# suilin0432/SoS-WSOD

Measured on AMD Instinct MI355X. Metric: images/s (1/2/4/8 MI355X) VGG16+OICR 2000-prop; conv5_3 MFMA-util %, higher is better.
Workload: dtype bf16; 1 GPU; OICR+ training iteration: 4 views/step/GPU (1 image(s) x 2 scales x h-flip, every view 512x512), R=2000 proposals/view, K=20, VGG16 dilated-C5 + ROIPool 7x7 + fc6/fc7 4096 + WSDDN + 4 OICR heads, fwd+bwd+SGD(momentum, wd); image=one view, parallelism=dp1

## Files before the change

### include/soswsod_hip.h

```cpp
#ifndef SOSWSOD_HIP_H
#define SOSWSOD_HIP_H

#include <stdint.h>

#ifdef __cplusplus
extern "C" {
#endif

#ifndef SW_F32
#define SW_F32 0
#define SW_BF16 1
#endif

typedef struct ihipStream_t* sw_stream_t;

typedef struct sw_epilogue {
  const float* bias;
  int relu;
  const uint8_t* drop_mask;
  long ld_drop;
  float drop_scale;
  const void* relu_ref;
  long ld_ref;
  float ref_scale;
  int ref_dtype;
  int out_dtype;
  int accumulate_atomic;
  float* absmax_out;
  uint64_t drop_seed, drop_offset;
  float drop_hash_p;
  const uint64_t* drop_offset_dev;
  float* splitk_workspace;
  const void* residual;
  long ld_res;
  int res_dtype;
  const float* fold_row_scale;
  const struct sw_sgd_tensor_s* sgd_fused;
  float sgd_momentum, sgd_grad_scale;
} sw_epilogue;

int sw_gemm(int dtype, int a_kstrided, int b_kstrided, int M, int N, int K, const void* A, long lda, const void* B,
            long ldb, void* C, long ldc, const sw_epilogue* ep, int splitk, sw_stream_t stream);
long sw_gemm_splitk_workspace_floats(int M, int N, int K, int splitk);

int sw_conv3x3_igemm(int dtype, int nimg, int H, int W, int Cin, int Cout, int dilation, const void* in,
                     const void* wk, void* out, const sw_epilogue* ep, sw_stream_t stream);
int sw_conv3x3_relu_pool2(int dtype, int nimg, int H, int W, int Cin, int Cout, const void* in, const void* wk, const float* bias,
                          void* out_pooled, sw_stream_t stream);
typedef struct sw_conv_problem {
  int32_t nimg, H, W, Cin, Cout;
  const void* in; const void* wk; void* out;
  const sw_epilogue* ep;
} sw_conv_problem;
int sw_conv3x3_multi(int dtype, int n, const sw_conv_problem* probs, sw_stream_t stream);
long sw_conv3x3_wgrad_workspace_floats(int dtype, int nimg, int H, int W, int Cin, int Cout, int splitk);
int sw_conv3x3_wgrad(int dtype, int nimg, int H, int W, int Cin, int Cout, int dilation, const void* x,
                     const void* dy, float* dw_oihw, float* workspace, int splitk, sw_stream_t stream);
int sw_conv3x3_wgrad_scaled(int dtype, int nimg, int H, int W, int Cin, int Cout, int dilation, const void* x, const void* dy,
                            float* dw_oihw, float* workspace, int splitk, const float* cout_scale, sw_stream_t stream);
int sw_conv3x3_wgrad_acc(int dtype, int nimg, int H, int W, int Cin, int Cout, int dilation, const void* x, const void* dy,
                         float* dw_oihw, float* workspace, int splitk, const float* cout_scale, int accumulate, sw_stream_t stream);
int sw_conv3x3_wgrad_small(int dtype, int nimg, int H, int W, int Cin, int Cout, const void* x, const void* dy,
                           const float* cout_scale, float* dw_oihw, sw_stream_t stream);
int sw_conv3x3_wgrad_small_acc(int dtype, int nimg, int H, int W, int Cin, int Cout, const void* x, const void* dy,
                               const float* cout_scale, float* dw_oihw, int accumulate, sw_stream_t stream);
int sw_conv3x3_wgrad_slabs(int dtype, int nimg, int H, int W, int Cin, int Cout, int dilation, const void* x,
                           const void* dy, float* workspace, int splitk, sw_stream_t stream);
int sw_conv3x3_wgrad_fold(int Cin, int Cout, int nslab, const float* workspace, float* dw_oihw, sw_stream_t stream);
int sw_conv3x3_wgrad_fold_acc(int Cin, int Cout, int nslab, const float* workspace, float* dw_oihw, const float* cout_scale,
                              int accumulate, sw_stream_t stream);
typedef struct {
  int nimg, H, W, Cin, Cout, dilation, nsplit;
  const void* x;
  const void* dy;
  float* slabs;
} sw_wgrad_problem;
int sw_conv3x3_wgrad_grouped(int dtype, int n_problems, const sw_wgrad_problem* problems, sw_stream_t stream);
typedef struct sw_gemm_kk_problem {
  const void* A; const void* B; float* slabs;
  int32_t M, N, K, nsplit;
  long lda, ldb;
} sw_gemm_kk_problem;
int sw_gemm_kk_grouped(int dtype, int n_problems, const sw_gemm_kk_problem* problems, sw_stream_t stream);
long sw_gemm_kk_grouped_slabs(int dtype, int K, int nsplit);
typedef struct sw_splitk_fold { int32_t M, N, nslab, accumulate; const float* workspace; float* C; long ldc; const float* row_scale; } sw_splitk_fold;
int sw_splitk_fold_multi(int n, const sw_splitk_fold* folds, sw_stream_t stream);
typedef struct { int Cin, Cout, nslab; const float* workspace; float* dw_oihw; } sw_wgrad_fold;
int sw_conv3x3_wgrad_fold_multi(int n, const sw_wgrad_fold* folds, sw_stream_t stream);
int sw_conv_weight_prep(int dtype, int mode, int Cout, int Cin, int cin_pad, const float* w_oihw, void* wk,
                        sw_stream_t stream);

int sw_maxpool2x2_fwd(int dtype, int nimg, int H, int W, int C, int stride, const void* in, void* out,
                      sw_stream_t stream);
int sw_maxpool2x2_bwd(int dtype, int nimg, int H, int W, int C, int stride, const void* in, const void* dout,
                      void* din, int relu_mask, sw_stream_t stream);
// ... 260 lines not shown
```

### sos-wsod_amd/_lib.py

```python
import ctypes
import os

import torch

_HERE = os.path.dirname(os.path.abspath(__file__))
LIB_PATH = os.environ.get("SW_LIB_PATH") or os.path.join(_HERE, "libsoswsod_hip.so")

SW_F32, SW_BF16 = 0, 1

c_int, c_long, c_float, c_void_p, c_u64 = ctypes.c_int, ctypes.c_long, ctypes.c_float, ctypes.c_void_p, ctypes.c_uint64


class Epilogue(ctypes.Structure):
    _fields_ = [
        ("bias", c_void_p), ("relu", c_int), ("drop_mask", c_void_p), ("ld_drop", c_long), ("drop_scale", c_float),
        ("relu_ref", c_void_p), ("ld_ref", c_long), ("ref_scale", c_float), ("ref_dtype", c_int),
        ("out_dtype", c_int), ("accumulate_atomic", c_int), ("absmax_out", c_void_p),
        ("drop_seed", c_u64), ("drop_offset", c_u64), ("drop_hash_p", c_float), ("drop_offset_dev", c_void_p),
        ("splitk_workspace", c_void_p),
        ("residual", c_void_p), ("ld_res", c_long), ("res_dtype", c_int),
        ("fold_row_scale", c_void_p),
        ("sgd_fused", c_void_p), ("sgd_momentum", c_float), ("sgd_grad_scale", c_float),
    ]

# ... 20 lines not shown
    _fields_ = [("src", ctypes.c_void_p), ("out", ctypes.c_void_p), ("tmp", ctypes.c_void_p), ("lsum", ctypes.c_void_p),
                ("H", ctypes.c_int32), ("W", ctypes.c_int32), ("recipe", AugRecipe)]


class GemmKKProblem(ctypes.Structure):
    _fields_ = [("A", ctypes.c_void_p), ("B", ctypes.c_void_p), ("slabs", ctypes.c_void_p), ("M", ctypes.c_int32), ("N", ctypes.c_int32),
                ("K", ctypes.c_int32), ("nsplit", ctypes.c_int32), ("lda", ctypes.c_long), ("ldb", ctypes.c_long)]


class SplitkFold(ctypes.Structure):
    _fields_ = [("M", ctypes.c_int32), ("N", ctypes.c_int32), ("nslab", ctypes.c_int32), ("accumulate", ctypes.c_int32),
                ("workspace", ctypes.c_void_p), ("C", ctypes.c_void_p), ("ldc", ctypes.c_long), ("row_scale", ctypes.c_void_p)]


class ConvProblem(ctypes.Structure):
    _fields_ = [("nimg", ctypes.c_int32), ("H", ctypes.c_int32), ("W", ctypes.c_int32), ("Cin", ctypes.c_int32), ("Cout", ctypes.c_int32),
                ("in_", ctypes.c_void_p), ("wk", ctypes.c_void_p), ("out", ctypes.c_void_p), ("ep", ctypes.POINTER(Epilogue))]


class CopyDesc(ctypes.Structure):
    _fields_ = [("src", ctypes.c_void_p), ("dst", ctypes.c_void_p), ("bytes", ctypes.c_long)]


class ColsumPart(ctypes.Structure):
    _fields_ = [("M", c_int), ("N", c_int), ("X", c_void_p), ("ld", c_long), ("workspace", c_void_p)]


class StageDesc(ctypes.Structure):
    _fields_ = [("w", c_void_p), ("bn_weight", c_void_p), ("bn_bias", c_void_p), ("bn_mean", c_void_p), ("bn_var", c_void_p),
                ("scale", c_void_p), ("shift", c_void_p), ("dst", c_void_p),
                ("kind", ctypes.c_int32), ("rows", ctypes.c_int32), ("cols", ctypes.c_int32), ("block_start", ctypes.c_int32)]


class ColsumFold(ctypes.Structure):
    _fields_ = [("N", ctypes.c_int), ("n_partial_rows", ctypes.c_int), ("workspace", ctypes.c_void_p), ("out", ctypes.c_void_p)]


class SgdTensor(ctypes.Structure):
    _fields_ = [
        ("param", c_void_p), ("grad", c_void_p), ("momentum_buf", c_void_p), ("n", c_long), ("lr", c_float),
        ("weight_decay", c_float), ("first_step", c_int), ("stage_kind", c_int), ("stage_dtype", c_int),
        ("stage0", c_void_p), ("stage1", c_void_p), ("d0", c_int), ("d1", c_int), ("d2", c_int), ("ld0", c_long), ("ld1", c_long),
        ("hyper_dev", c_void_p),
    ]


SGD_MAX_TENSORS = 24
_EP = ctypes.POINTER(Epilogue)
_F4 = ctypes.POINTER(c_float)

SIGNATURES = {
    "sw_gemm": (c_int, [c_int, c_int, c_int, c_int, c_int, c_int, c_void_p, c_long, c_void_p, c_long, c_void_p, c_long,
                        _EP, c_int, c_void_p]),
    "sw_gemm_splitk_workspace_floats": (c_long, [c_int, c_int, c_int, c_int]),
    "sw_gemm_sgd_fused_supported": (c_int, [c_int, c_int, c_int, c_int, c_int, c_int]),
    "sw_conv3x3_igemm": (c_int, [c_int, c_int, c_int, c_int, c_int, c_int, c_int, c_void_p, c_void_p, c_void_p, _EP,
                                 c_void_p]),
    "sw_conv3x3_wgrad": (c_int, [c_int, c_int, c_int, c_int, c_int, c_int, c_int, c_void_p, c_void_p, c_void_p, c_void_p,
                                 c_int, c_void_p]),
    "sw_conv3x3_wgrad_workspace_floats": (c_long, [c_int, c_int, c_int, c_int, c_int, c_int, c_int]),
    "sw_conv_weight_prep": (c_int, [c_int, c_int, c_int, c_int, c_int, c_void_p, c_void_p, c_void_p]),
    "sw_maxpool2x2_fwd": (c_int, [c_int, c_int, c_int, c_int, c_int, c_int, c_void_p, c_void_p, c_void_p]),
    "sw_maxpool2x2_bwd": (c_int, [c_int, c_int, c_int, c_int, c_int, c_int, c_void_p, c_void_p, c_void_p, c_int,
                                  c_void_p]),
    "sw_preprocess": (c_int, [c_int, c_int, c_int, c_int, c_void_p, _F4, _F4, c_void_p, c_void_p]),
    "sw_preprocess_multi": (c_int, [c_int, c_int, c_int, c_int, c_int, ctypes.POINTER(c_void_p), _F4, _F4, c_void_p, c_void_p]),
    "sw_roi_pool_fwd": (c_int, [c_int, c_int, c_int, c_int, c_int, c_int, c_int, c_float, c_void_p, c_void_p, c_int,
                                c_void_p, c_float, c_void_p, c_void_p, c_int, c_long, c_void_p]),
    "sw_roi_pool_fwd_workspace_bytes": (c_long, [c_int, c_int, c_int, c_int]),
    "sw_roi_pool_fwd_ws": (c_int, [c_int, c_int, c_int, c_int, c_int, c_int, c_int, c_float, c_void_p, c_void_p, c_int,
                                   c_void_p, c_float, c_void_p, c_void_p, c_int, c_long, c_void_p, c_long, c_void_p]),
    "sw_roi_pool_bwd": (c_int, [c_int, c_int, c_int, c_int, c_int, c_int, c_int, c_void_p, c_void_p, c_int, c_long, c_void_p, c_int,
                                c_void_p, c_float, c_void_p, c_void_p, c_void_p, c_float, c_void_p]),
    "sw_absmax": (c_int, [c_int, c_long, c_void_p, c_void_p, c_void_p]),
    "sw_wsddn_workspace_floats": (c_long, [c_int, c_int, c_int]),
    "sw_wsddn_mil": (c_int, [c_int, c_int, c_int, c_void_p, c_long, c_int, c_int, c_void_p, c_void_p, c_void_p,
                             c_void_p, c_long, c_void_p, c_void_p, c_long, c_void_p, c_void_p]),
    "sw_mean_views": (c_int, [c_int, c_long, c_void_p, c_void_p, c_void_p]),
    "sw_oicr_mean_probs": (c_int, [c_int, c_int, c_int, c_int, c_void_p, c_long, c_int, c_int, c_void_p, c_void_p]),
    "sw_mine_workspace_bytes": (c_long, [c_int, c_int, c_int]),
    "sw_oicr_mine_label": (c_int, [c_int, c_int, c_int, c_int, c_void_p, c_void_p, c_int, c_void_p, c_int, c_float, c_float,
                                   c_float, c_float, c_void_p, c_void_p, c_void_p, c_void_p, c_void_p, c_void_p,
                                   c_void_p, c_void_p, c_void_p]),
    "sw_oicr_refine_loss": (c_int, [c_int, c_int, c_int, c_int, c_void_p, c_long, c_int, c_int, c_int, c_void_p, c_void_p,
                                    c_void_p, c_void_p, c_void_p, _F4, c_void_p, c_void_p, c_long, c_void_p,
                                    c_void_p, c_void_p]),
    "sw_oicr_predict": (c_int, [c_int, c_int, c_int, c_void_p, c_long, c_int, c_int, c_void_p, _F4, c_float, c_void_p,
                                c_void_p, c_void_p]),
    "sw_detect_workspace_bytes": (c_long, [c_int, c_int]),
    "sw_detect_postprocess": (c_int, [c_int, c_int, c_void_p, c_void_p, c_int, c_int, c_float, c_float, c_int, c_void_p,
                                      c_void_p, c_void_p, c_void_p, c_void_p, c_void_p, c_void_p]),
    "sw_detect_workspace_bytes2": (c_long, [c_int, c_int, c_int]),
    "sw_detect_postprocess2": (c_int, [c_int, c_int, c_void_p, c_void_p, c_int, c_int, c_float, c_float, c_int, c_void_p,
                                       c_void_p, c_void_p, c_void_p, c_void_p, c_void_p, c_long, c_void_p]),
    "sw_colsum": (c_int, [c_int, c_int, c_int, c_void_p, c_long, c_void_p, c_void_p, c_void_p]),
    "sw_colsum_acc": (c_int, [c_int, c_int, c_int, c_void_p, c_long, c_void_p, c_void_p, c_int, c_void_p]),
    "sw_colsum_workspace_floats": (c_long, [c_int, c_int, c_int]),
    "sw_colsum_partial": (c_int, [c_int, c_int, c_int, c_void_p, c_long, c_void_p, c_void_p]),
    "sw_colsum_fold": (c_int, [c_int, c_int, c_void_p, c_void_p, c_void_p]),
    "sw_conv3x3_wgrad_scaled": (c_int, [c_int, c_int, c_int, c_int, c_int, c_int, c_int, c_void_p, c_void_p, c_void_p, c_void_p, c_int,
                                        c_void_p, c_void_p]),
    "sw_conv3x3_wgrad_acc": (c_int, [c_int, c_int, c_int, c_int, c_int, c_int, c_int, c_void_p, c_void_p, c_void_p, c_void_p, c_int,
                                     c_void_p, c_int, c_void_p]),
    "sw_conv3x3_wgrad_small": (c_int, [c_int, c_int, c_int, c_int, c_int, c_int, c_void_p, c_void_p, c_void_p, c_void_p, c_void_p]),
    "sw_conv3x3_wgrad_small_acc": (c_int, [c_int, c_int, c_int, c_int, c_int, c_int, c_void_p, c_void_p, c_void_p, c_void_p, c_int, c_void_p]),
    "sw_conv3x3_wgrad_slabs": (c_int, [c_int, c_int, c_int, c_int, c_int, c_int, c_int, c_void_p, c_void_p, c_void_p, c_int,
# ... 126 lines not shown
```

### sos-wsod_amd/csrc/gemm.hip

```cpp
#include "common.h"
#include "soswsod_hip.h"

namespace {

enum { OP_KCONTIG = 0, OP_KSTRIDED = 1, OP_CONV_A = 2, OP_CONV_B = 3, OP_CONV_A_GEN = 4 };

struct GemmArgs {
  const void* A; const void* B; void* C;
  int M, N, K;
  long lda, ldb, ldc;
  int tiles_m, tiles_n, patches_m, k_per_split;
  int patch_m_log2;
  int cH, cW, cC, cDil;
  const float* bias;
  const uint8_t* drop; long ldd; float drop_scale;
  unsigned long long drop_seed_mixed, drop_offset; float drop_p;
  const unsigned long long* drop_offset_dev;
  const void* ref; long ldr; float ref_scale; int ref_bf16;
  const void* res; long ldres; int res_bf16;
  int relu, out_bf16, atomic, oihw_cin, staged_out;
  unsigned a_bytes, b_bytes;
  long slab_stride;
  int vgrid;
  int krot;
// ... 631 lines not shown
        if (g.slab_stride > 0) __builtin_nontemporal_store(v, (float*)g.C + o + (long)zsplit * g.slab_stride);
        else if (g.atomic) atomicAdd((float*)g.C + o, v);
        else if (g.out_bf16) __builtin_nontemporal_store(f32_to_bf16_bits(v), (unsigned short*)g.C + o);
        else __builtin_nontemporal_store(v, (float*)g.C + o);
      }
    }
  if (staged) {
    constexpr int CPRW = WTN / 8;
#pragma unroll
    for (int q = 0; q < (WTM * CPRW) / 64; ++q) {
      const int idx = q * 64 + lane, lrow = idx / CPRW, ch = idx % CPRW;
      const int m = m0 + wm * WTM + lrow, n = n0t + wn * WTN + ch * 8;
      if (m < g.M && n < g.N) {
        __builtin_nontemporal_store(*(const u32x4*)(stile + lrow * WTN + ch * 8), (u32x4*)((unsigned short*)g.C + (long)m * g.ldc + n));
      }
    }
  }
  }
  if (g.absmax) {
    vmax = wave_reduce_max_u32(vmax);
    if (lane == 0) atomicMax((unsigned int*)g.absmax, vmax);
  }
}

template <typename T, int AMODE, int BMODE, int BM, int BN, int STAGES, int WTM, int WTN>
__global__ __launch_bounds__((BM / WTM) * (BN / WTN) * 64, 1) void gemm2_kernel(GemmArgs g) {
  extern __shared__ __attribute__((aligned(16))) char smem[];
  const int vgrid = (g.vgrid > 0 && gridDim.z == 1) ? g.vgrid : (int)gridDim.x;
  for (int vbid = blockIdx.x; vbid < vgrid; vbid += gridDim.x) {
  int bm, bn, zsplit = 0;
  if (gridDim.z > 1) {
    const int ntv = gridDim.x, tot = ntv * (int)gridDim.z;
    const int f = blockIdx.z * ntv + blockIdx.x;
    const int x = f & 7, j = f >> 3;
    const int w = x * (tot >> 3) + min(x, tot & 7) + j;
    zsplit = w / ntv;
    const int t = w - zsplit * ntv;
    bm = t % g.tiles_m; bn = t / g.tiles_m;
  } else {
    const int nwg = vgrid;
    const int bid = vbid;
    const int swz = (bid & 7) * (nwg >> 3) + (bid >> 3);
    const int patch = swz >> 6, within = swz & 63;
    const int pml = g.patch_m_log2;
    bm = ((patch % g.patches_m) << pml) + (within & ((1 << pml) - 1));
    bn = ((patch / g.patches_m) << (6 - pml)) + (within >> pml);
    if (bm >= g.tiles_m || bn >= g.tiles_n) continue;
  }
  gemm2_tile<T, AMODE, BMODE, BM, BN, STAGES, WTM, WTN>(g, bm, bn, zsplit, smem);
  if (vbid + (int)gridDim.x < vgrid) __syncthreads();
  }
}

struct GroupedProblem {
  const void* A; const void* B; float* C;
  int M, N, K, cH, cW, cC, cDil, k_per_split, nsplit, tiles_m, tiles_n;
  unsigned a_bytes, b_bytes;
  int lda, ldb;
};
constexpr int GROUPED_MAX = 40;
struct GroupedArgs {
  int n_problems, n_items;
  int first_item[GROUPED_MAX + 1];
  GroupedProblem p[GROUPED_MAX];
};

template <typename T, int BMODE = OP_CONV_B>
__global__ __launch_bounds__(1024, 1) void gemm2_grouped_kernel(GroupedArgs ga) {
  extern __shared__ __attribute__((aligned(16))) char smem[];
  const int G = gridDim.x;
  for (int vbid = blockIdx.x; vbid < ga.n_items; vbid += G) {
    const int round = vbid / G, within = vbid - round * G;
    const int in_round = min(G, ga.n_items - round * G);
    const int x = within & 7, j = within >> 3;
    const int per = in_round >> 3, extra = in_round & 7;
    if (j >= per + (x < extra ? 1 : 0)) continue;
    const int t = round * G + x * per + min(x, extra) + j;
    int pi = 0;
    while (pi + 1 < ga.n_problems && t >= ga.first_item[pi + 1]) ++pi;
    const GroupedProblem& P = ga.p[pi];
    const int local = t - ga.first_item[pi];
    const int ntile = P.tiles_m * P.tiles_n;
    const int zsplit = local / ntile, tl = local - zsplit * ntile;
    GemmArgs g = {};
    g.A = P.A; g.B = P.B; g.C = P.C; g.M = P.M; g.N = P.N; g.K = P.K; g.lda = P.lda; g.ldb = P.ldb; g.ldc = P.N;
    g.cH = P.cH; g.cW = P.cW; g.cC = P.cC; g.cDil = P.cDil; g.k_per_split = P.k_per_split;
    g.tiles_m = P.tiles_m; g.tiles_n = P.tiles_n; g.a_bytes = P.a_bytes; g.b_bytes = P.b_bytes;
    g.slab_stride = (long)P.M * P.N; g.drop_scale = 1.f; g.ref_scale = 1.f;
    gemm2_tile<T, OP_KSTRIDED, BMODE, 256, 256, 2, 64, 64>(g, tl % P.tiles_m, tl / P.tiles_m, zsplit, smem);
    __syncthreads();
  }
}


template <typename T, int AMODE, int BMODE, int BM, int BN, int STAGES, int WTM = 64, int WTN = 64>
int launch2(GemmArgs& g, int splitk, hipStream_t stream) {
  constexpr int BK = GT<T>::BK;
  using GA = Geom2<T, AMODE, BM>;
  using GB = Geom2<T, BMODE, BN>;
  constexpr int LDS = STAGES * (GA::BYTES + GB::BYTES);
  constexpr int NT = (BM / WTM) * (BN / WTN) * 64;
  g.tiles_m = (g.M + BM - 1) / BM;
  g.tiles_n = (g.N + BN - 1) / BN;
  int pml = 3;
  if (g.tiles_n < 8) { int l = 0; while ((1 << l) < g.tiles_n) ++l; pml = 6 - l; }
  else if (g.tiles_m < 8) { int l = 0; while ((1 << l) < g.tiles_m) ++l; pml = l; }
  g.patch_m_log2 = pml;
  g.patches_m = (g.tiles_m + (1 << pml) - 1) >> pml;
  const int patches_n = (g.tiles_n + (64 >> pml) - 1) / (64 >> pml);
  if (splitk < 1) splitk = 1;
  int kps = (g.K + splitk - 1) / splitk;
  kps = ((kps + BK - 1) / BK) * BK;
  g.k_per_split = kps;
  splitk = (g.K + kps - 1) / kps;
  if (splitk > 1 && !g.atomic && g.slab_stride <= 0) return -2;
  g.staged_out = (g.out_bf16 && !g.atomic && g.slab_stride <= 0 && (g.N % 8) == 0 && (g.ldc % 8) == 0 &&
                  (((uintptr_t)g.C) & 15) == 0 && (long)NT / 64 * WTM * WTN * 2 <= (long)LDS) ? 1 : 0;
  if (BM == 256 && BN == 256 && WTM == 128 && WTN == 64 && sizeof(T) == 2)
    g.staged_out = ((((uintptr_t)g.C) & 15) == 0 && (g.ldc % (g.out_bf16 && g.slab_stride <= 0 ? 8 : 4)) == 0 &&
                    (g.slab_stride % 4) == 0) ? 1 : 0;
  dim3 grid(splitk > 1 ? g.tiles_m * g.tiles_n : g.patches_m * patches_n * 64, 1, splitk), block(NT);
  const int ncu = sw_cu_count();
  if ((ncu % 8) == 0 && splitk == 1 && BM == 256 && BN == 256 && (int)grid.x > ncu) { g.vgrid = (int)grid.x; grid.x = ncu; }
  auto kern = gemm2_kernel<T, AMODE, BMODE, BM, BN, STAGES, WTM, WTN>;
  hipError_t e = hipFuncSetAttribute((const void*)kern, hipFuncAttributeMaxDynamicSharedMemorySize, LDS);
  if (e != hipSuccess) return (int)e;
  hipLaunchKernelGGL(kern, grid, block, LDS, stream, g);
  SW_CHECK_LAUNCH();
  return 0;
}

template <typename T, int AMODE, int BMODE>
int launch_auto(GemmArgs& g, int splitk, hipStream_t s) {
  const long sk = splitk < 1 ? 1 : splitk;
  auto tiles = [&](int bm, int bn) { return (long)((g.M + bm - 1) / bm) * ((g.N + bn - 1) / bn) * sk; };
  if (g.N > 128 && tiles(256, 256) >= 200 && g.K >= 1024) {
    if constexpr (sizeof(T) == 2 && AMODE == OP_KCONTIG && BMODE <= OP_KSTRIDED) {
      if ((g.K % 64) == 0 && sk == 1) return launch2<T, AMODE, BMODE, 256, 256, 2, 128, 64>(g, splitk, s);
    }
    return launch2<T, AMODE, BMODE, 256, 256, 2>(g, splitk, s);
  }
  if (g.N <= 64 && sk == 1) return launch2<T, AMODE, BMODE, 256, 64, 2, 32, 64>(g, splitk, s);
  if constexpr (sizeof(T) == 2 && AMODE <= OP_KSTRIDED && BMODE <= OP_KSTRIDED) {
    if (tiles(128, 128) <= 256 && g.K >= 512) return launch2<T, AMODE, BMODE, 128, 128, 4, 32, 64>(g, splitk, s);
  }
  return launch2<T, AMODE, BMODE, 128, 128, 2, 32, 64>(g, splitk, s);
}

template <typename T>
int dispatch_modes(GemmArgs& g, int amode, int bmode, int splitk, hipStream_t s) {
  if (amode == OP_KCONTIG && bmode == OP_KCONTIG) return launch_auto<T, OP_KCONTIG, OP_KCONTIG>(g, splitk, s);
  if (amode == OP_KCONTIG && bmode == OP_KSTRIDED) return launch_auto<T, OP_KCONTIG, OP_KSTRIDED>(g, splitk, s);
  if (amode == OP_KSTRIDED && bmode == OP_KSTRIDED) return launch_auto<T, OP_KSTRIDED, OP_KSTRIDED>(g, splitk, s);
  if (amode == OP_CONV_A && bmode == OP_KCONTIG) return launch_auto<T, OP_CONV_A, OP_KCONTIG>(g, splitk, s);
  if (amode == OP_CONV_A_GEN && bmode == OP_KCONTIG) return launch_auto<T, OP_CONV_A_GEN, OP_KCONTIG>(g, splitk, s);
  if (amode == OP_KSTRIDED && bmode == OP_CONV_B) return launch_auto<T, OP_KSTRIDED, OP_CONV_B>(g, splitk, s);
  return -3;
}

__global__ void scale_rows_kernel(int M, int N, float* __restrict__ C, long ldc, const float* __restrict__ row_scale) {
  const long total = (long)M * N;
  for (long i = blockIdx.x * (long)blockDim.x + threadIdx.x; i < total; i += (long)gridDim.x * blockDim.x) {
    const long m = i / N;
    float* p = C + m * ldc + (i - m * N);
    *p = __fmul_rn(*p, row_scale[m]);
  }
}

__global__ __launch_bounds__(256) void splitk_reduce_kernel(int M, int N, int nslab, const float* __restrict__ ws,
                                                            float* __restrict__ C, long ldc, int vec, const float* __restrict__ row_scale) {
  const long slab = (long)M * N;
  if (vec) {
    const long nv = slab >> 2;
    const int nq = N >> 2;
    for (long q = blockIdx.x * (long)blockDim.x + threadIdx.x; q < nv; q += (long)gridDim.x * blockDim.x) {
      const f32x4* src = (const f32x4*)ws + q;
      f32x4 a0 = {0.f, 0.f, 0.f, 0.f}, a1 = a0, a2 = a0, a3 = a0;
      int z = 0;
      for (; z + 4 <= nslab; z += 4) {
        const f32x4 v0 = src[(long)z * nv], v1 = src[(long)(z + 1) * nv], v2 = src[(long)(z + 2) * nv], v3 = src[(long)(z + 3) * nv];
        a0 += v0; a1 += v1; a2 += v2; a3 += v3;
// ... 69 lines not shown
      *(f32x4*)((float*)f.C + m * f.ldc + n) = o;
    }
  }
}

bool peel_geometry(int M, int N, int* r_out, long* sk_out) {
  const long tm = (M + 255) / 256, tn = (N + 255) / 256, tiles = tm * tn;
  if (!(tiles >= 512 && (tiles % 256) != 0 && (tiles % 256) <= 160)) return false;
  int r = 0;
  for (int c = 1; c <= 4 && !r; ++c)
    if (tn - c >= 2 && (tm * (tn - c)) % 256 == 0) r = c;
  if (!r) return false;
  const int N2 = N - (int)((tn - r) * 256);
  const long t128 = ((M + 127) / 128) * ((N2 + 127) / 128);
  long sk = 512 / t128;
  sk = sk < 1 ? 1 : (sk > 8 ? 8 : sk);
  while (sk > 1 && tm * r * sk >= 200) --sk;
  *r_out = r; *sk_out = sk;
  return true;
}

int effective_splits(int dtype, int K, int splitk) {
  const int bk = dtype == SW_BF16 ? 64 : 32;
  if (splitk < 1) splitk = 1;
  int kps = (K + splitk - 1) / splitk;
  kps = ((kps + bk - 1) / bk) * bk;
  return (K + kps - 1) / kps;
}

int check_align(const void* p) { return (((uintptr_t)p) & 15) ? -4 : 0; }

}

int sw_sgd_tile_t_block(int rows, int cols, float* param, const float* grad, float* buf, long ld_src, float lr, float wd, int first,
                        float mom, float gscale, unsigned short* st0, long ld0, unsigned short* st1, long ld1, const float* hyper,
                        hipStream_t stream);

static bool sgd_fused_shape_ok(int dtype, int a_kstrided, int b_kstrided, int M, int N, int K) {
  if (dtype != SW_BF16 || a_kstrided) return false;
  (void)b_kstrided;
  if ((M % 64) || (N % 64) || (K % 64) || K < 1024 || N <= 128) return false;
  return ((long)((M + 255) / 256) * ((N + 255) / 256)) >= 200;
}
static bool sgd_fused_accepts(int dtype, int a_kstrided, int b_kstrided, int M, int N, int K) {
  if (!sgd_fused_shape_ok(dtype, a_kstrided, b_kstrided, M, N, K)) return false;
  int r = 0; long sk = 1;
  if (!peel_geometry(M, N, &r, &sk)) return true;
  const int N1 = (int)(((N + 255) / 256 - r) * 256);
  return sgd_fused_shape_ok(dtype, a_kstrided, b_kstrided, M, N1, K) && ((N - N1) % 64) == 0;
}
extern "C" int sw_gemm_sgd_fused_supported(int dtype, int a_kstrided, int b_kstrided, int M, int N, int K) {
  return sgd_fused_accepts(dtype, a_kstrided, b_kstrided, M, N, K) ? 1 : 0;
}

extern "C" int sw_gemm(int dtype, int a_kstrided, int b_kstrided, int M, int N, int K, const void* A, long lda,
                       const void* B, long ldb, void* C, long ldc, const sw_epilogue* ep, int splitk,
                       hipStream_t stream) {
  SW_ENTER();
  if (M <= 0 || N <= 0 || K <= 0) return 0;
  const int epc = dtype == SW_BF16 ? 8 : 4;
  if (dtype != SW_BF16 && dtype != SW_F32) return -1;
  if (check_align(A) || check_align(B)) return -4;
  if ((lda % epc) || (ldb % epc)) return -5;
  if (!a_kstrided && (K % epc)) return -5;
  if (!b_kstrided && (K % epc)) return -5;
  if (a_kstrided && (M % epc)) return -5;
  if (b_kstrided && (N % epc)) return -5;
  if (a_kstrided && !b_kstrided) return -3;
  const bool plain = (!ep || (ep->out_dtype == SW_F32 && !ep->bias && !ep->relu && !ep->drop_mask && !(ep->drop_hash_p > 0.f) && !ep->relu_ref &&
                              !ep->accumulate_atomic && !ep->absmax_out && !ep->residual));
  const bool has_row_scale = ep && ep->fold_row_scale;
  float* const det_ws = (ep && plain) ? ep->splitk_workspace : nullptr;
  {
    int r = 0; long sk = 1;
    if (plain && !has_row_scale && splitk <= 1 && peel_geometry(M, N, &r, &sk)) {
      const long es = dtype == SW_BF16 ? 2 : 4;
      const long tn = (N + 255) / 256;
      const int N1 = (int)((tn - r) * 256), N2 = N - N1;
      const char* B2 = (const char*)B + (b_kstrided ? (long)N1 * es : (long)N1 * ldb * es);
      sw_epilogue ep1 = {};
      ep1.out_dtype = SW_F32; ep1.drop_scale = 1.f; ep1.ref_scale = 1.f;
      const sw_sgd_tensor* fz = ep ? ep->sgd_fused : nullptr;
      if (fz) {
        if (!sgd_fused_accepts(dtype, a_kstrided, b_kstrided, M, N, K) || !fz->stage1) return -5;
        ep1.sgd_fused = fz; ep1.sgd_momentum = ep->sgd_momentum; ep1.sgd_grad_scale = ep->sgd_grad_scale;
      }
      int rc = sw_gemm(dtype, a_kstrided, b_kstrided, M, N1, K, A, lda, B, ldb, C, ldc, &ep1, 1, stream);
      if (rc) return rc;
      float* C2 = (float*)C + N1;
      ep1.sgd_fused = nullptr;
      sw_epilogue ep2 = ep1;
      if (det_ws) ep2.splitk_workspace = det_ws;
      else if (sk > 1) {
        hipError_t e = hipMemset2DAsync(C2, (size_t)ldc * 4, 0, (size_t)N2 * 4, (size_t)M, stream);
        if (e != hipSuccess) return (int)e;
        ep2.accumulate_atomic = 1;
      }
      rc = sw_gemm(dtype, a_kstrided, b_kstrided, M, N2, K, A, lda, B2, ldb, C2, ldc, &ep2, (int)sk, stream);
      if (rc || !fz) return rc;
      return sw_sgd_tile_t_block(M, N2, fz->param + N1, C2, fz->momentum_buf + N1, ldc, fz->lr, fz->weight_decay, fz->first_step,
                                 ep->sgd_momentum, ep->sgd_grad_scale, fz->stage0 ? (unsigned short*)fz->stage0 + N1 : nullptr, fz->ld0,
                                 (unsigned short*)fz->stage1 + (long)N1 * fz->ld1, fz->ld1, fz->hyper_dev, stream);
    }
  }
  if (ep && ep->sgd_fused) {
    const sw_sgd_tensor* fz = ep->sgd_fused;
    if (!plain || splitk > 1 || !sgd_fused_accepts(dtype, a_kstrided, b_kstrided, M, N, K)) return -5;
    if (fz->stage_kind != 3 || fz->stage_dtype != SW_BF16 || !fz->stage1 || fz->d0 < N || !fz->param || !fz->momentum_buf) return -5;
    if ((ldc % 4) || (fz->ld0 % 4) || (fz->ld1 % 8) || ((((uintptr_t)fz->param) | ((uintptr_t)fz->momentum_buf)) & 15) ||
        (((uintptr_t)fz->stage0) & 7) || (((uintptr_t)fz->stage1) & 15)) return -4;
  }
  const int eff = effective_splits(dtype, K, splitk);
  const bool fold_ep = ep && !plain && (eff > 1 || (ep->fold_row_scale && ep->residual)) && ep->splitk_workspace &&
                       !ep->accumulate_atomic && !ep->drop_mask && !(ep->drop_hash_p > 0.f) && !ep->absmax_out;
  if (fold_ep) {
    if ((N % 4) || (ldc % 4) || (((uintptr_t)C) & 7) || (((uintptr_t)ep->splitk_workspace) & 15)) return -5;
    if (ep->residual && ((ep->ld_res % 4) || (((uintptr_t)ep->residual) & 7))) return -5;
    float* const slabs = ep->splitk_workspace;
    GemmArgs gs = {};
    gs.A = A; gs.B = B; gs.M = M; gs.N = N; gs.K = K; gs.lda = lda; gs.ldb = ldb;
    gs.C = slabs; gs.ldc = N; gs.slab_stride = (long)M * N; gs.drop_scale = 1.f; gs.ref_scale = 1.f;
    {
      const long es = dtype == SW_BF16 ? 2 : 4;
      const long ab = (long)(a_kstrided ? K : M) * lda * es, bb = (long)(b_kstrided ? K : N) * ldb * es;
      if (ab >= 0xFFFFFF00L || bb >= 0xFFFFFF00L) return -6;
      gs.a_bytes = (unsigned)ab; gs.b_bytes = (unsigned)bb;
    }
    const int am = a_kstrided ? OP_KSTRIDED : OP_KCONTIG, bmo = b_kstrided ? OP_KSTRIDED : OP_KCONTIG;
    const int rc = dtype == SW_BF16 ? dispatch_modes<unsigned short>(gs, am, bmo, eff, stream) : dispatch_modes<float>(gs, am, bmo, eff, stream);
    if (rc) return rc;
    FoldEp f = {};
    f.M = M; f.N = N; f.nslab = eff; f.ws = slabs; f.C = C; f.ldc = ldc; f.out_bf16 = ep->out_dtype == SW_BF16;
    f.bias = ep->bias; f.row_scale = ep->fold_row_scale;
    f.res = ep->residual; f.ldres = ep->ld_res; f.res_bf16 = ep->res_dtype == SW_BF16;
    f.relu = ep->relu; f.ref = ep->relu_ref; f.ldr = ep->ld_ref; f.ref_bf16 = ep->ref_dtype == SW_BF16; f.ref_scale = ep->ref_scale;
    long blocks = (((long)M * N >> 2) + 255) / 256;
    blocks = blocks < 1 ? 1 : (blocks > 4096 ? 4096 : blocks);
    hipLaunchKernelGGL(splitk_fold_ep_kernel, dim3((unsigned)blocks), dim3(256), 0, stream, f);
    SW_CHECK_LAUNCH();
    return 0;
  }
  const bool det = det_ws != nullptr && eff > 1;
  if (det && (((uintptr_t)det_ws) & 15)) return -4;
  GemmArgs g = {};
  g.A = A; g.B = B; g.C = C; g.M = M; g.N = N; g.K = K; g.lda = lda; g.ldb = ldb; g.ldc = ldc;
  if (ep) {
    g.bias = ep->bias; g.drop = ep->drop_mask; g.ldd = ep->ld_drop; g.drop_scale = ep->drop_scale;
    g.ref = ep->relu_ref; g.ldr = ep->ld_ref; g.ref_scale = ep->ref_scale; g.ref_bf16 = ep->ref_dtype == SW_BF16;
    g.res = ep->residual; g.ldres = ep->ld_res; g.res_bf16 = ep->res_dtype == SW_BF16;
    g.relu = ep->relu; g.out_bf16 = ep->out_dtype == SW_BF16; g.atomic = ep->accumulate_atomic; g.absmax = ep->absmax_out;
    if (ep->sgd_fused) {
      const sw_sgd_tensor* fz = ep->sgd_fused;
      g.sgd_param = fz->param; g.sgd_mom = fz->momentum_buf; g.sgd_ld = ldc;
      g.sgd_st0 = (unsigned short*)fz->stage0; g.sgd_ld0 = fz->ld0; g.sgd_st1 = (unsigned short*)fz->stage1; g.sgd_ld1 = fz->ld1;
      g.sgd_hyper = fz->hyper_dev; g.sgd_lr = fz->lr; g.sgd_wd = fz->weight_decay; g.sgd_first = fz->first_step;
      g.sgd_momentum = ep->sgd_momentum; g.sgd_gscale = ep->sgd_grad_scale;
    }
    if (!ep->drop_mask && ep->drop_hash_p > 0.f) {
      unsigned long long x = ep->drop_seed;
      x += 0x9E3779B97F4A7C15ull;
      x = (x ^ (x >> 30)) * 0xBF58476D1CE4E5B9ull;
      x = (x ^ (x >> 27)) * 0x94D049BB133111EBull;
      x ^= x >> 31;
      g.drop_seed_mixed = x; g.drop_offset = ep->drop_offset; g.drop_p = ep->drop_hash_p;
      g.drop_offset_dev = (const unsigned long long*)ep->drop_offset_dev;
    }
  }
  {
    const long es = dtype == SW_BF16 ? 2 : 4;
    const long ab = (long)(a_kstrided ? K : M) * lda * es, bb = (long)(b_kstrided ? K : N) * ldb * es;
    if (ab >= 0xFFFFFF00L || bb >= 0xFFFFFF00L) return -6;
    g.a_bytes = (unsigned)ab; g.b_bytes = (unsigned)bb;
  }
  const int am = a_kstrided ? OP_KSTRIDED : OP_KCONTIG, bmo = b_kstrided ? OP_KSTRIDED : OP_KCONTIG;
  if (det) {
    g.C = det_ws; g.ldc = N; g.slab_stride = (long)M * N; g.atomic = 0;
  }
  const int rc = dtype == SW_BF16 ? dispatch_modes<unsigned short>(g, am, bmo, det ? eff : splitk, stream)
                                  : dispatch_modes<float>(g, am, bmo, det ? eff : splitk, stream);
  if (rc) return rc;
  if (!det) {
    if (ep && ep->fold_row_scale) {
      if (!plain || ep->out_dtype != SW_F32) return -5;
      long blocks = ((long)M * N + 255) / 256;
      blocks = blocks > 4096 ? 4096 : blocks;
      hipLaunchKernelGGL(scale_rows_kernel, dim3((unsigned)blocks), dim3(256), 0, stream, M, N, (float*)C, ldc, ep->fold_row_scale);
      SW_CHECK_LAUNCH();
    }
    return 0;
  }
  const int vec = ((N % 4) == 0 && (ldc % 4) == 0 && (((uintptr_t)C) & 15) == 0) ? 1 : 0;
  long blocks = (((long)M * N >> (vec ? 2 : 0)) + 255) / 256;
  blocks = blocks < 1 ? 1 : (blocks > 4096 ? 4096 : blocks);
  hipLaunchKernelGGL(splitk_reduce_kernel, dim3((unsigned)blocks), dim3(256), 0, stream, M, N, eff, det_ws, (float*)C, ldc, vec,
                     ep ? ep->fold_row_scale : nullptr);
  SW_CHECK_LAUNCH();
  return 0;
}

extern "C" long sw_gemm_splitk_workspace_floats(int M, int N, int K, int splitk) {
  if (M <= 0 || N <= 0 || K <= 0) return 0;
  if (splitk > 1) return (long)splitk * M * N;
  int r = 0; long sk = 1;
  if (peel_geometry(M, N, &r, &sk) && sk > 1) {
    const long tn = (N + 255) / 256;
    const int N2 = N - (int)((tn - r) * 256);
    return sk * (long)M * N2;
  }
  return 0;
}

int sw_conv3x3_direct_try(int nimg, int H, int W, int Cin, int Cout, int dilation, const void* in, const void* wk, void* out,
                          const sw_epilogue* ep, hipStream_t stream);

extern "C" int sw_conv3x3_igemm(int dtype, int nimg, int H, int W, int Cin, int Cout, int dilation, const void* in,
                                const void* wk, void* out, const sw_epilogue* ep, hipStream_t stream) {
  SW_ENTER();
  const int epc = dtype == SW_BF16 ? 8 : 4;
  if (dtype != SW_BF16 && dtype != SW_F32) return -1;
  if (Cin % epc) return -5;
  if (check_align(in) || check_align(wk)) return -4;
  if (dtype == SW_BF16) {
    const int rc = sw_conv3x3_direct_try(nimg, H, W, Cin, Cout, dilation, in, wk, out, ep, stream);
    if (rc != 0) return rc < 0 ? -rc : 0;
  }
  GemmArgs g = {};
  g.A = in; g.B = wk; g.C = out; g.M = nimg * H * W; g.N = Cout; g.K = 9 * Cin; g.lda = 0; g.ldb = 9L * Cin; g.ldc = Cout;
  g.cH = H; g.cW = W; g.cC = Cin; g.cDil = dilation;
  g.krot = dtype == SW_BF16 ? 1 : 0;
  if (ep) {
    g.bias = ep->bias; g.drop = ep->drop_mask; g.ldd = ep->ld_drop; g.drop_scale = ep->drop_scale;
    g.ref = ep->relu_ref; g.ldr = ep->ld_ref; g.ref_scale = ep->ref_scale; g.ref_bf16 = ep->ref_dtype == SW_BF16;
    g.relu = ep->relu; g.out_bf16 = ep->out_dtype == SW_BF16; g.atomic = ep->accumulate_atomic;
  }
  {
    const long es = dtype == SW_BF16 ? 2 : 4;
    const long ab = (long)nimg * H * W * Cin * es, bb = (long)Cout * 9 * Cin * es;
    if (ab >= 0xFFFFFF00L || bb >= 0xFFFFFF00L) return -6;
    g.a_bytes = (unsigned)ab; g.b_bytes = (unsigned)bb;
  }
  const int bk = dtype == SW_BF16 ? 64 : 32;
  const int amode = (Cin % bk == 0) ? OP_CONV_A : OP_CONV_A_GEN;
  return dtype == SW_BF16 ? dispatch_modes<unsigned short>(g, amode, OP_KCONTIG, 1, stream)
                          : dispatch_modes<float>(g, amode, OP_KCONTIG, 1, stream);
}

namespace {
__device__ __forceinline__ void wgrad_reduce_body(int Cout, int Cin, int nslab, const float* __restrict__ slabs,
                                                  float* __restrict__ out, int co, int parts, int part, float* s_t,
                                                  const float* __restrict__ cout_scale = nullptr, const int accumulate = 0) {
// ... 347 lines not shown
```

### sos-wsod_amd/ops.py

```python
import ctypes
import os

import torch

from ._lib import SW_BF16, SW_F32, Epilogue, check, lib


def _p(t):
    return None if t is None else ctypes.c_void_p(t.data_ptr())


_raw_stream = getattr(torch._C, "_cuda_getCurrentRawStream", None)


def _stream():
    if _raw_stream is not None:
        return ctypes.c_void_p(_raw_stream(torch.cuda.current_device()))
    return ctypes.c_void_p(torch.cuda.current_stream().cuda_stream)


def dt(t_or_dtype):
    d = t_or_dtype if isinstance(t_or_dtype, torch.dtype) else t_or_dtype.dtype
    if d == torch.float32:
        return SW_F32
# ... 172 lines not shown


def _drop_staging(key):
    ent = STAGING.get(key)
    if ent is not None and ent["param"]() is None:
        STAGING.pop(key, None)


def _launch(tag, fn):
    if TIMER is None or tag is None:
        return fn()
    return TIMER.wrap(tag, fn)


def _need_gpu(*ts):
    for t in ts:
        if t is not None and not t.is_cuda:
            raise RuntimeError("sos-wsod_amd kernels need GPU tensors (there is no CPU fallback)")


def make_epilogue(bias=None, relu=False, drop_mask=None, drop_scale=2.0, relu_ref=None, ref_scale=1.0,
                  out_dtype=torch.float32, atomic=False, absmax_out=None, drop_hash=None, splitk_workspace=None, residual=None,
                  row_scale=None):
    ep = Epilogue()
    ep.bias = None if bias is None else bias.data_ptr()
    ep.relu = int(relu)
    ep.drop_mask = None if drop_mask is None else drop_mask.data_ptr()
    ep.ld_drop = 0 if drop_mask is None else drop_mask.stride(0)
    ep.drop_scale = float(drop_scale)
    if relu_ref is not None and relu_ref.dim() != 2:
        raise ValueError("relu_ref: a (rows, columns) matrix (its row pitch is the reference's leading dimension)")
    ep.relu_ref = None if relu_ref is None else relu_ref.data_ptr()
    ep.ld_ref = 0 if relu_ref is None else relu_ref.stride(0)
    ep.ref_scale = float(ref_scale)
    ep.ref_dtype = SW_F32 if relu_ref is None else dt(relu_ref)
    ep.out_dtype = dt(out_dtype)
    ep.accumulate_atomic = int(atomic)
    ep.absmax_out = None if absmax_out is None else absmax_out.data_ptr()
    ep.splitk_workspace = None if splitk_workspace is None else splitk_workspace.data_ptr()
    if drop_hash is not None and drop_mask is None:
        ep.drop_seed, ep.drop_offset, ep.drop_hash_p = int(drop_hash[0]) & (2 ** 64 - 1), int(drop_hash[1]), float(drop_hash[2])
        if len(drop_hash) > 3 and drop_hash[3] is not None:
            ep.drop_offset_dev = drop_hash[3].data_ptr()
    if residual is not None and residual.dim() != 2:
        raise ValueError("residual: a (rows, columns) matrix")
    ep.residual = None if residual is None else residual.data_ptr()
    ep.ld_res = 0 if residual is None else residual.stride(0)
    ep.res_dtype = SW_F32 if residual is None else dt(residual)
    ep.fold_row_scale = None if row_scale is None else row_scale.data_ptr()
    ep._keepalive = (bias, drop_mask, relu_ref, absmax_out, splitk_workspace, drop_hash, residual, row_scale)
    return ep


def gemm(A, B, C, M, N, K, a_kstrided=False, b_kstrided=False, lda=None, ldb=None, ldc=None, ep=None, splitk=1, tag=None):
    _need_gpu(A, B, C)
    lda = A.stride(0) if lda is None else lda
    ldb = B.stride(0) if ldb is None else ldb
    ldc = C.stride(0) if ldc is None else ldc
    if ep is None:
        ep = make_epilogue(out_dtype=C.dtype)
    if (C.dtype == torch.float32 or splitk > 1) and not ep.accumulate_atomic and not ep.splitk_workspace:
        need = int(lib.sw_gemm_splitk_workspace_floats(M, N, K, splitk))
        if need > 0:
            ws = torch.empty(need, device=C.device, dtype=torch.float32)
            ep.splitk_workspace = ws.data_ptr()
            ep._keepalive = ep._keepalive + (ws,)
    check(_launch(tag, lambda: lib.sw_gemm(dt(A), int(a_kstrided), int(b_kstrided), M, N, K, _p(A), lda, _p(B), ldb, _p(C),
                                           ldc, ctypes.byref(ep), splitk, _stream())), "sw_gemm")
    return C


def conv3x3(x, wk, out, dilation, ep, tag=None):
    _need_gpu(x, wk, out)
    n, H, W, Cin = x.shape
    Cout = out.shape[3]
    if TIMER is not None and tag is not None:
        TIMER.note(tag, 2.0 * n * H * W * Cout * 9 * Cin)
    check(_launch(tag, lambda: lib.sw_conv3x3_igemm(dt(x), n, H, W, Cin, Cout, dilation, _p(x), _p(wk), _p(out),
                                                    ctypes.byref(ep), _stream())), "sw_conv3x3_igemm")
    return out


def conv3x3_relu_pool2(x, wk, bias, out_pooled, tag=None):
    _need_gpu(x, wk, out_pooled)
    n, H, W, Cin = x.shape
    Cout = out_pooled.shape[3]
    if TIMER is not None and tag is not None:
        TIMER.note(tag, 2.0 * n * H * W * Cout * 9 * Cin)
    rc = _launch(tag, lambda: lib.sw_conv3x3_relu_pool2(dt(x), n, H, W, Cin, Cout, _p(x), _p(wk), _p(bias), _p(out_pooled), _stream()))
    if rc < 0:
        check(rc, "sw_conv3x3_relu_pool2")
    return rc == 1


def conv3x3_multi(problems):
    from ._lib import ConvProblem
    n = len(problems)
    if n == 0:
        return
    if 1 < n <= 8 and problems[0][0].dtype == torch.bfloat16:
        arr = (ConvProblem * n)()
        for i, (x, wk, out, ep) in enumerate(problems):
            _need_gpu(x, wk, out)
            q = arr[i]
            q.nimg, q.H, q.W, q.Cin = x.shape
            q.Cout = out.shape[3]
            q.in_, q.wk, q.out, q.ep = x.data_ptr(), wk.data_ptr(), out.data_ptr(), ctypes.pointer(ep)
        rc = int(lib.sw_conv3x3_multi(SW_BF16, n, arr, _stream()))
        if rc == 1:
            return
        if rc < 0:
            check(rc, "sw_conv3x3_multi")
    for x, wk, out, ep in problems:
        conv3x3(x, wk, out, 1, ep)


def conv3x3_wgrad(x, dy, dw_oihw, dilation, splitk=1, workspace=None, tag=None, cout_scale=None, accumulate=False):
    _need_gpu(x, dy, dw_oihw)
    n, H, W, Cin = x.shape
# ... 1052 lines not shown
```

Before: 509.9 images/s.

## Fuse split GEMM halves into one persistent dephased kernel with SGD epilogue

When the fused-SGD GEMM is split into a main part and a split-K tail, both are now scheduled in one persistent kernel sized to the CU count. Half the workgroups start on tail pieces first so the work is staggered across CUs. This removes a separate launch and the tail's underutilised wave, at the cost of more complex scheduling and per-workgroup work imbalance. The new path runs when the default sw_gemm hits the split-N fused-SGD case (resident=0 falls back to the CU count).

```diff
diff --git a/include/soswsod_hip.h b/include/soswsod_hip.h
--- a/include/soswsod_hip.h
+++ b/include/soswsod_hip.h
@@ -41,6 +41,8 @@
 
 int sw_gemm(int dtype, int a_kstrided, int b_kstrided, int M, int N, int K, const void* A, long lda, const void* B,
             long ldb, void* C, long ldc, const sw_epilogue* ep, int splitk, sw_stream_t stream);
+int sw_gemm_resident(int dtype, int a_kstrided, int b_kstrided, int M, int N, int K, const void* A, long lda, const void* B,
+                     long ldb, void* C, long ldc, const sw_epilogue* ep, int splitk, int resident_workgroups, sw_stream_t stream);
 long sw_gemm_splitk_workspace_floats(int M, int N, int K, int splitk);
 
 int sw_conv3x3_igemm(int dtype, int nimg, int H, int W, int Cin, int Cout, int dilation, const void* in,
diff --git a/sos-wsod_amd/_lib.py b/sos-wsod_amd/_lib.py
--- a/sos-wsod_amd/_lib.py
+++ b/sos-wsod_amd/_lib.py
@@ -96,6 +96,8 @@
 SIGNATURES = {
     "sw_gemm": (c_int, [c_int, c_int, c_int, c_int, c_int, c_int, c_void_p, c_long, c_void_p, c_long, c_void_p, c_long,
                         _EP, c_int, c_void_p]),
+    "sw_gemm_resident": (c_int, [c_int, c_int, c_int, c_int, c_int, c_int, c_void_p, c_long, c_void_p, c_long, c_void_p, c_long,
+                                 _EP, c_int, c_int, c_void_p]),
     "sw_gemm_splitk_workspace_floats": (c_long, [c_int, c_int, c_int, c_int]),
     "sw_gemm_sgd_fused_supported": (c_int, [c_int, c_int, c_int, c_int, c_int, c_int]),
     "sw_conv3x3_igemm": (c_int, [c_int, c_int, c_int, c_int, c_int, c_int, c_int, c_void_p, c_void_p, c_void_p, _EP,
diff --git a/sos-wsod_amd/csrc/gemm.hip b/sos-wsod_amd/csrc/gemm.hip
--- a/sos-wsod_amd/csrc/gemm.hip
+++ b/sos-wsod_amd/csrc/gemm.hip
@@ -707,6 +707,49 @@
   }
 }
 
+struct DephasedArgs {
+  GemmArgs g;
+  GemmArgs t;
+  int t_pieces, t_tiles, t_first;
+};
+
+template <typename T, int AMODE, int BMODE, int BM, int BN, int STAGES, int WTM, int WTN>
+__global__ __launch_bounds__((BM / WTM) * (BN / WTN) * 64, 1) void gemm2_dephased_kernel(DephasedArgs d) {
+  extern __shared__ __attribute__((aligned(16))) char smem[];
+  const int G = gridDim.x, b = blockIdx.x;
+  const int x = b & 7, slot = b >> 3;
+  const bool shifted = (slot & 1) != 0;
+  const int nA = ((G >> 3) >> 1) << 3, nB = G - nA;
+  const int rank = shifted ? x * (nA >> 3) + (slot >> 1) : x * (nB >> 3) + (slot >> 1);
+  const int n_first = min(d.t_pieces, d.t_first * nA);
+  const int n_late = d.t_pieces - n_first;
+  const int my_first = (shifted && rank < n_first) ? (n_first - rank + nA - 1) / nA : 0;
+  const int my_main = b < d.g.vgrid ? (d.g.vgrid - b + G - 1) / G : 0;
+  const int late_rank = shifted ? nB + rank : rank;
+  const int my_late = late_rank < n_late ? (n_late - late_rank + G - 1) / G : 0;
+  for (int it = 0; it < my_first + my_main + my_late; ++it) {
+    const bool tail = it < my_first || it >= my_first + my_main;
+    const GemmArgs& g = tail ? d.t : d.g;
+    int bm, bn, zsplit = 0;
+    if (tail) {
+      const int p = it < my_first ? rank + it * nA : n_first + late_rank + (it - my_first - my_main) * G;
+      zsplit = p / d.t_tiles;
+      const int tl = p - zsplit * d.t_tiles;
+      bm = tl % g.tiles_m; bn = tl / g.tiles_m;
+    } else {
+      const int bid = b + (it - my_first) * G;
+      const int swz = (bid & 7) * (g.vgrid >> 3) + (bid >> 3);
+      const int patch = swz >> 6, within = swz & 63;
+      const int pml = g.patch_m_log2;
+      bm = ((patch % g.patches_m) << pml) + (within & ((1 << pml) - 1));
+      bn = ((patch / g.patches_m) << (6 - pml)) + (within >> pml);
+      if (bm >= g.tiles_m || bn >= g.tiles_n) continue;
+    }
+    gemm2_tile<T, AMODE, BMODE, BM, BN, STAGES, WTM, WTN>(g, bm, bn, zsplit, smem);
+    __syncthreads();
+  }
+}
+
 struct GroupedProblem {
   const void* A; const void* B; float* C;
   int M, N, K, cH, cW, cC, cDil, k_per_split, nsplit, tiles_m, tiles_n;
@@ -748,8 +791,8 @@
 }
 
 
-template <typename T, int AMODE, int BMODE, int BM, int BN, int STAGES, int WTM = 64, int WTN = 64>
-int launch2(GemmArgs& g, int splitk, hipStream_t stream) {
+template <typename T, int AMODE, int BMODE, int BM, int BN, int STAGES, int WTM, int WTN>
+int plan2(GemmArgs& g, int splitk, int* patched_wgs) {
   constexpr int BK = GT<T>::BK;
   using GA = Geom2<T, AMODE, BM>;
   using GB = Geom2<T, BMODE, BN>;
@@ -774,7 +817,20 @@
   if (BM == 256 && BN == 256 && WTM == 128 && WTN == 64 && sizeof(T) == 2)
     g.staged_out = ((((uintptr_t)g.C) & 15) == 0 && (g.ldc % (g.out_bf16 && g.slab_stride <= 0 ? 8 : 4)) == 0 &&
                     (g.slab_stride % 4) == 0) ? 1 : 0;
-  dim3 grid(splitk > 1 ? g.tiles_m * g.tiles_n : g.patches_m * patches_n * 64, 1, splitk), block(NT);
+  *patched_wgs = g.patches_m * patches_n * 64;
+  return splitk;
+}
+
+template <typename T, int AMODE, int BMODE, int BM, int BN, int STAGES, int WTM = 64, int WTN = 64>
+int launch2(GemmArgs& g, int splitk, hipStream_t stream) {
+  using GA = Geom2<T, AMODE, BM>;
+  using GB = Geom2<T, BMODE, BN>;
+  constexpr int LDS = STAGES * (GA::BYTES + GB::BYTES);
+  constexpr int NT = (BM / WTM) * (BN / WTN) * 64;
+  int patched = 0;
+  splitk = plan2<T, AMODE, BMODE, BM, BN, STAGES, WTM, WTN>(g, splitk, &patched);
+  if (splitk < 0) return splitk;
+  dim3 grid(splitk > 1 ? g.tiles_m * g.tiles_n : patched, 1, splitk), block(NT);
   const int ncu = sw_cu_count();
   if ((ncu % 8) == 0 && splitk == 1 && BM == 256 && BN == 256 && (int)grid.x > ncu) { g.vgrid = (int)grid.x; grid.x = ncu; }
   auto kern = gemm2_kernel<T, AMODE, BMODE, BM, BN, STAGES, WTM, WTN>;
@@ -782,6 +838,29 @@
   if (e != hipSuccess) return (int)e;
   hipLaunchKernelGGL(kern, grid, block, LDS, stream, g);
   SW_CHECK_LAUNCH();
+  return 0;
+}
+
+int launch_dephased(GemmArgs& g, GemmArgs& t, int t_splits, int resident, hipStream_t stream, bool* launched) {
+  *launched = false;
+  using T = unsigned short;
+  constexpr int AM = OP_KCONTIG, BMD = OP_KSTRIDED, LDS = 2 * (Geom2<T, AM, 256>::BYTES + Geom2<T, BMD, 256>::BYTES);
+  const int G = resident > 0 ? resident : sw_cu_count();
+  if ((G % 8) || G < 16) return 0;
+  int wgs = 0, t_wgs = 0;
+  if (plan2<T, AM, BMD, 256, 256, 2, 128, 64>(g, 1, &wgs) != 1 || wgs <= G) return 0;
+  if (plan2<T, AM, BMD, 256, 256, 2, 128, 64>(t, t_splits, &t_wgs) != t_splits) return 0;
+  g.vgrid = wgs;
+  DephasedArgs d;
+  d.g = g; d.t = t;
+  d.t_tiles = t.tiles_m * t.tiles_n; d.t_pieces = d.t_tiles * t_splits;
+  d.t_first = t_splits / 2 > 1 ? t_splits / 2 : 1;
+  auto kern = gemm2_dephased_kernel<T, AM, BMD, 256, 256, 2, 128, 64>;
+  hipError_t e = hipFuncSetAttribute((const void*)kern, hipFuncAttributeMaxDynamicSharedMemorySize, LDS);
+  if (e != hipSuccess) return (int)e;
+  hipLaunchKernelGGL(kern, dim3(G), dim3(512), LDS, stream, d);
+  SW_CHECK_LAUNCH();
+  *launched = true;
   return 0;
 }
 
@@ -957,11 +1036,16 @@
 extern "C" int sw_gemm_sgd_fused_supported(int dtype, int a_kstrided, int b_kstrided, int M, int N, int K) {
   return sgd_fused_accepts(dtype, a_kstrided, b_kstrided, M, N, K) ? 1 : 0;
 }
-
-extern "C" int sw_gemm(int dtype, int a_kstrided, int b_kstrided, int M, int N, int K, const void* A, long lda,
-                       const void* B, long ldb, void* C, long ldc, const sw_epilogue* ep, int splitk,
-                       hipStream_t stream) {
-  SW_ENTER();
+static int sgd_fused_tensor_check(const sw_sgd_tensor* fz, int N, long ldc) {
+  if (fz->stage_kind != 3 || fz->stage_dtype != SW_BF16 || !fz->stage1 || fz->d0 < N || !fz->param || !fz->momentum_buf) return -5;
+  if ((ldc % 4) || (fz->ld0 % 4) || (fz->ld1 % 8) || ((((uintptr_t)fz->param) | ((uintptr_t)fz->momentum_buf)) & 15) ||
+      (((uintptr_t)fz->stage0) & 7) || (((uintptr_t)fz->stage1) & 15)) return -4;
+  return 0;
+}
+
+static int gemm_impl(int dtype, int a_kstrided, int b_kstrided, int M, int N, int K, const void* A, long lda,
+                     const void* B, long ldb, void* C, long ldc, const sw_epilogue* ep, int splitk, int resident,
+                     hipStream_t stream) {
   if (M <= 0 || N <= 0 || K <= 0) return 0;
   const int epc = dtype == SW_BF16 ? 8 : 4;
   if (dtype != SW_BF16 && dtype != SW_F32) return -1;
@@ -990,9 +1074,41 @@
         if (!sgd_fused_accepts(dtype, a_kstrided, b_kstrided, M, N, K) || !fz->stage1) return -5;
         ep1.sgd_fused = fz; ep1.sgd_momentum = ep->sgd_momentum; ep1.sgd_grad_scale = ep->sgd_grad_scale;
       }
-      int rc = sw_gemm(dtype, a_kstrided, b_kstrided, M, N1, K, A, lda, B, ldb, C, ldc, &ep1, 1, stream);
+      float* C2 = (float*)C + N1;
+      const int eff2 = effective_splits(dtype, K, (int)sk);
+      if (fz && b_kstrided && (det_ws || eff2 == 1)) {
+        if (const int rc = sgd_fused_tensor_check(fz, N1, ldc)) return rc;
+        if (eff2 > 1 && (((uintptr_t)det_ws) & 15)) return -4;
+        const long ab = (long)M * lda * es, bb = (long)K * ldb * es;
+        if (ab >= 0xFFFFFF00L || bb >= 0xFFFFFF00L) return -6;
+        GemmArgs g = {}, t = {};
+        g.A = A; g.B = B; g.C = C; g.M = M; g.N = N1; g.K = K; g.lda = lda; g.ldb = ldb; g.ldc = ldc;
+        g.drop_scale = 1.f; g.ref_scale = 1.f; g.a_bytes = (unsigned)ab; g.b_bytes = (unsigned)bb;
+        t = g;
+        t.B = B2; t.N = N2;
+        if (eff2 > 1) { t.C = det_ws; t.ldc = N2; t.slab_stride = (long)M * N2; } else t.C = C2;
+        g.sgd_param = fz->param; g.sgd_mom = fz->momentum_buf; g.sgd_ld = ldc;
+        g.sgd_st0 = (unsigned short*)fz->stage0; g.sgd_ld0 = fz->ld0; g.sgd_st1 = (unsigned short*)fz->stage1; g.sgd_ld1 = fz->ld1;
+        g.sgd_hyper = fz->hyper_dev; g.sgd_lr = fz->lr; g.sgd_wd = fz->weight_decay; g.sgd_first = fz->first_step;
+        g.sgd_momentum = ep->sgd_momentum; g.sgd_gscale = ep->sgd_grad_scale;
+        bool launched = false;
+        if (const int rc = launch_dephased(g, t, eff2, resident, stream, &launched)) return rc;
+        if (launched) {
+          if (eff2 > 1) {
+            const int vec = ((N2 % 4) == 0 && (ldc % 4) == 0 && (((uintptr_t)C2) & 15) == 0) ? 1 : 0;
+            long blocks = (((long)M * N2 >> (vec ? 2 : 0)) + 255) / 256;
+            blocks = blocks < 1 ? 1 : (blocks > 4096 ? 4096 : blocks);
+            hipLaunchKernelGGL(splitk_reduce_kernel, dim3((unsigned)blocks), dim3(256), 0, stream, M, N2, eff2, det_ws, C2, ldc, vec,
+                               (const float*)nullptr);
+            SW_CHECK_LAUNCH();
+          }
+          return sw_sgd_tile_t_block(M, N2, fz->param + N1, C2, fz->momentum_buf + N1, ldc, fz->lr, fz->weight_decay, fz->first_step,
+                                     ep->sgd_momentum, ep->sgd_grad_scale, fz->stage0 ? (unsigned short*)fz->stage0 + N1 : nullptr,
+                                     fz->ld0, (unsigned short*)fz->stage1 + (long)N1 * fz->ld1, fz->ld1, fz->hyper_dev, stream);
+        }
+      }
+      int rc = gemm_impl(dtype, a_kstrided, b_kstrided, M, N1, K, A, lda, B, ldb, C, ldc, &ep1, 1, 0, stream);
       if (rc) return rc;
-      float* C2 = (float*)C + N1;
       ep1.sgd_fused = nullptr;
       sw_epilogue ep2 = ep1;
       if (det_ws) ep2.splitk_workspace = det_ws;
@@ -1001,7 +1117,7 @@
         if (e != hipSuccess) return (int)e;
         ep2.accumulate_atomic = 1;
       }
-      rc = sw_gemm(dtype, a_kstrided, b_kstrided, M, N2, K, A, lda, B2, ldb, C2, ldc, &ep2, (int)sk, stream);
+      rc = gemm_impl(dtype, a_kstrided, b_kstrided, M, N2, K, A, lda, B2, ldb, C2, ldc, &ep2, (int)sk, 0, stream);
       if (rc || !fz) return rc;
       return sw_sgd_tile_t_block(M, N2, fz->param + N1, C2, fz->momentum_buf + N1, ldc, fz->lr, fz->weight_decay, fz->first_step,
                                  ep->sgd_momentum, ep->sgd_grad_scale, fz->stage0 ? (unsigned short*)fz->stage0 + N1 : nullptr, fz->ld0,
@@ -1011,9 +1127,7 @@
   if (ep && ep->sgd_fused) {
     const sw_sgd_tensor* fz = ep->sgd_fused;
     if (!plain || splitk > 1 || !sgd_fused_accepts(dtype, a_kstrided, b_kstrided, M, N, K)) return -5;
-    if (fz->stage_kind != 3 || fz->stage_dtype != SW_BF16 || !fz->stage1 || fz->d0 < N || !fz->param || !fz->momentum_buf) return -5;
-    if ((ldc % 4) || (fz->ld0 % 4) || (fz->ld1 % 8) || ((((uintptr_t)fz->param) | ((uintptr_t)fz->momentum_buf)) & 15) ||
-        (((uintptr_t)fz->stage0) & 7) || (((uintptr_t)fz->stage1) & 15)) return -4;
+    if (const int rc = sgd_fused_tensor_check(fz, N, ldc)) return rc;
   }
   const int eff = effective_splits(dtype, K, splitk);
   const bool fold_ep = ep && !plain && (eff > 1 || (ep->fold_row_scale && ep->residual)) && ep->splitk_workspace &&
@@ -1101,6 +1215,21 @@
                      ep ? ep->fold_row_scale : nullptr);
   SW_CHECK_LAUNCH();
   return 0;
+}
+
+extern "C" int sw_gemm(int dtype, int a_kstrided, int b_kstrided, int M, int N, int K, const void* A, long lda,
+                       const void* B, long ldb, void* C, long ldc, const sw_epilogue* ep, int splitk,
+                       hipStream_t stream) {
+  SW_ENTER();
+  return gemm_impl(dtype, a_kstrided, b_kstrided, M, N, K, A, lda, B, ldb, C, ldc, ep, splitk, 0, stream);
+}
+
+extern "C" int sw_gemm_resident(int dtype, int a_kstrided, int b_kstrided, int M, int N, int K, const void* A, long lda,
+                                const void* B, long ldb, void* C, long ldc, const sw_epilogue* ep, int splitk,
+                                int resident_workgroups, hipStream_t stream) {
+  SW_ENTER();
+  if (resident_workgroups < 0) return -5;
+  return gemm_impl(dtype, a_kstrided, b_kstrided, M, N, K, A, lda, B, ldb, C, ldc, ep, splitk, resident_workgroups, stream);
 }
 
 extern "C" long sw_gemm_splitk_workspace_floats(int M, int N, int K, int splitk) {
diff --git a/sos-wsod_amd/ops.py b/sos-wsod_amd/ops.py
--- a/sos-wsod_amd/ops.py
+++ b/sos-wsod_amd/ops.py
@@ -248,7 +248,8 @@
     return ep
 
 
-def gemm(A, B, C, M, N, K, a_kstrided=False, b_kstrided=False, lda=None, ldb=None, ldc=None, ep=None, splitk=1, tag=None):
+def gemm(A, B, C, M, N, K, a_kstrided=False, b_kstrided=False, lda=None, ldb=None, ldc=None, ep=None, splitk=1, tag=None,
+         resident=0):
     _need_gpu(A, B, C)
     lda = A.stride(0) if lda is None else lda
     ldb = B.stride(0) if ldb is None else ldb
@@ -261,6 +262,10 @@
             ws = torch.empty(need, device=C.device, dtype=torch.float32)
             ep.splitk_workspace = ws.data_ptr()
             ep._keepalive = ep._keepalive + (ws,)
+    if resident:
+        check(_launch(tag, lambda: lib.sw_gemm_resident(dt(A), int(a_kstrided), int(b_kstrided), M, N, K, _p(A), lda, _p(B), ldb,
+                                                        _p(C), ldc, ctypes.byref(ep), splitk, int(resident), _stream())), "sw_gemm")
+        return C
     check(_launch(tag, lambda: lib.sw_gemm(dt(A), int(a_kstrided), int(b_kstrided), M, N, K, _p(A), lda, _p(B), ldb, _p(C),
                                            ldc, ctypes.byref(ep), splitk, _stream())), "sw_gemm")
     return C
```

Result: no change. 509.7 images/s (-0.0%).
